# zzzzxxxx111/Rover-SLAM

Hardware: AMD Instinct MI355X
Metric: frames/s SuperPoint+LightGlue 640x480 (higher is better)
Workload: dtype f32; 1 GPU; configs[3] per GPU: 33 synthetic 640x480 u8 frames resident in HBM, SuperPoint extract (Kmax=1024, thr=0.0005) + LightGlue match of 32 consecutive pairs (9 layers, filter 0.1); 32 frames counted per GPU per step; seeded synthetic weights (centred descriptor head + calibrated LightGlue law, frames shifted by multiples of 8 px); the same resident frames every step (compute-bound path, no data-depend; frames_per_gpu=32, kmax=1024, lg_fold_wo=1, pairing=calibrated

## Files before the change

rover-slam_amd/csrc/gemm.hip:

```cpp
#include <stdlib.h>
#include "rfe_internal.h"

namespace rfe {

constexpr int BK = 32, LDT = BK + 1;

__device__ __forceinline__ float gelu_short(float t) {
    const float x = t * 0.70710678118654752f, ax = fabsf(x);
    const float k = __builtin_amdgcn_rcpf(fmaf(0.3275911f, ax, 1.0f));
    const float poly = fmaf(fmaf(fmaf(fmaf(1.061405429f, k, -1.453152027f), k, 1.421413741f), k, -0.284496736f), k, 0.254829592f) * k;
    const float er = 1.0f - poly * __builtin_amdgcn_exp2f(-(ax * ax) * 1.44269504088896341f);
    return 0.5f * t * (1.0f + copysignf(er, x));
}

typedef __attribute__((address_space(3))) void* gemm_lds_ptr_t;
typedef const __attribute__((address_space(1))) void* gemm_gptr_t;
template <int MB, int NB, bool RES, bool LNA = false, bool KP = false, bool ROPE = false>
__global__ __launch_bounds__(256, 2) void gemm_nt_kernel(GemmArgs g) {
    constexpr int BM = MB * 64, BN = NB * 64;
    constexpr int LDR = KP ? BK : LDT;
    static_assert(!KP || (!LNA && MB == 2), "KP: 128-row tiles without the fused LayerNorm only");
    static_assert(!ROPE || (KP && !RES && NB == 4), "ROPE: plain k-permuted 128 x 256 tile only");
    __shared__ __attribute__((aligned(16))) float lds_static[(BM + BN) * LDR];
    extern __shared__ __attribute__((aligned(16))) float lds_dynamic[];
// ... 287 lines not shown
        if (i < T) {
            const int r = i & 15;
            const int m = m0 + (wm * MB + (i >> 4)) * 32 + (r & 3) + 8 * (r >> 2) + 4 * h;
            if (m < M) {
                const int P = (int)gridDim.x * 2;
                float* sp = g.stats_out + (((size_t)m + (size_t)z * g.M) * P + bxt * 2 + wn) * 2;
                sp[0] = sm[0]; sp[1] = s2[0];
            }
        }
    }
}

bool gemm_nt_rope_ok(const GemmArgs& g) {
    const int batch = g.batch > 0 ? g.batch : 1;
    return g.kperm && batch == 1 && !g.m_valid && !g.R && !g.stats_in && !g.stats_out && !g.Bh && !g.relu && g.alpha == 1.0f && g.N % 256 == 0 &&
           g.rope_c0 % 256 == 0 && g.rope_c1 % 256 == 0 && (long long)((g.M + 127) / 128) * (g.N / 256) >= 256 && !gemm_latency_regime(g);
}

int launch_gemm_nt(hipStream_t s, const GemmArgs& g_in) {
    GemmArgs g = g_in;
    const int batch = g.batch > 0 ? g.batch : 1;
    auto tiles = [&](int bm, int bn) { return (long long)((g.M + bm - 1) / bm) * ((g.N + bn - 1) / bn) * batch; };
    if (g.rope_csn && !gemm_nt_rope_ok(g)) return -1;
    if (g.Bh && g.Bl && batch == 1 && !g.m_valid && !g.relu && g.N % 256 == 0 && g.K % 32 == 0 && (!g.A2 || g.K1 % 32 == 0) && tiles(128, 256) >= 256)
        return launch_gemm_h2(s, g);
    if (!g.rope_csn && gemm_latency_regime(g)) {
        if (launch_gemm_lat(s, g, nullptr, 0)) return 0;
    }
    const bool res = g.R != nullptr, lna = g.stats_in != nullptr;
    const bool kp = g.kperm != 0 && !lna;
#define RFE_GEMM_GO(MB_, NB_, GRID)                                                                  \
    do {                                                                                             \
        if (g.rope_csn && MB_ == 2 && NB_ == 4) {                                                    \
            static bool lr_[64]; ensure_dynamic_lds((const void*)gemm_nt_kernel<2, 4, false, false, true, true>, 128 * 64 * 4, lr_); \
            hipLaunchKernelGGL((gemm_nt_kernel<2, 4, false, false, true, true>), GRID, dim3(256), 128 * 64 * 4, s, g); \
        } else                                                                                       \
        if (kp && MB_ == 2) {                                                                        \
            if (res) hipLaunchKernelGGL((gemm_nt_kernel<MB_, NB_, true, false, MB_ == 2>), GRID, dim3(256), 0, s, g); \
            else hipLaunchKernelGGL((gemm_nt_kernel<MB_, NB_, false, false, MB_ == 2>), GRID, dim3(256), 0, s, g);    \
        } else                                                                                       \
        if (lna) hipLaunchKernelGGL((gemm_nt_kernel<MB_, NB_, true, true>), GRID, dim3(256), 0, s, g);   \
        else if (res) hipLaunchKernelGGL((gemm_nt_kernel<MB_, NB_, true>), GRID, dim3(256), 0, s, g);    \
        else hipLaunchKernelGGL((gemm_nt_kernel<MB_, NB_, false>), GRID, dim3(256), 0, s, g);        \
    } while (0)
    const bool big = (g.N % 256 == 0 && tiles(128, 256) >= 256) || tiles(128, 128) >= 256 || g.M > 8192;
    if (!big || g.N % 256) g.stats_out = nullptr;
    int ntiles;
    if (g.N % 256 == 0 && tiles(128, 256) >= 256) { ntiles = g.N / 256; RFE_GEMM_GO(2, 4, dim3(g.N / 256, (g.M + 127) / 128, batch)); }
    else if (tiles(128, 128) >= 256 || g.M > 8192) { ntiles = (g.N + 127) / 128; RFE_GEMM_GO(2, 2, dim3((g.N + 127) / 128, (g.M + 127) / 128, batch)); }
    else if (tiles(64, 128) >= 256) { ntiles = (g.N + 127) / 128; RFE_GEMM_GO(1, 2, dim3((g.N + 127) / 128, (g.M + 63) / 64, batch)); }
    else { ntiles = (g.N + 63) / 64; RFE_GEMM_GO(1, 1, dim3((g.N + 63) / 64, (g.M + 63) / 64, batch)); }
    return g.stats_out ? 2 * ntiles : 0;
}

}
```

rover-slam_amd/csrc/lg_kernels.hip:

```cpp
#include <stdlib.h>
#include "rfe_internal.h"

namespace rfe {

__global__ void lg_posenc_kernel(const float* __restrict__ kn, const float* __restrict__ wr, int rows, float2* __restrict__ csn) {
    const int gid = blockIdx.x * blockDim.x + threadIdx.x;
    if (gid >= rows * 32) return;
    const int i = gid >> 5, f = gid & 31;
    const float th = fmaf(wr[2 * f + 1], kn[2 * i + 1], wr[2 * f] * kn[2 * i]);
    csn[gid] = make_float2(cosf(th), sinf(th));
}
void launch_lg_posenc(hipStream_t s, const float* kn, const float* wr, int rows, float* csn) {
    hipLaunchKernelGGL(lg_posenc_kernel, dim3((rows * 32 + 255) / 256), dim3(256), 0, s, kn, wr, rows, reinterpret_cast<float2*>(csn));
}

constexpr int AT_Q = 128, AT_K = 64, AT_LDK = 65;
constexpr float AT_DEFER = 16.0f;
constexpr int AT_SPLIT_MAX = 8;
constexpr size_t AT_SPLIT_MAX_ROWS = 8192;

__device__ __forceinline__ float at_softmax_init(bool first, float m_run) { return first ? 0.f : -m_run; }
__device__ __forceinline__ void at_softmax_step(f32x16& st, bool first, float& m_run, float& l_run, f32x16& o0, f32x16& o1) {
    float mx = fmaxf(fmaxf(st[0], st[1]), st[2]);
#pragma unroll
// ... 332 lines not shown
            acc.x += o.x * w; acc.y += o.y * w; acc.z += o.z * w; acc.w += o.w * w;
        }
        const float inv = l > 0.f ? 1.0f / l : 0.f;
        acc.x *= inv; acc.y *= inv; acc.z *= inv; acc.w *= inv;
    }
    *reinterpret_cast<float4*>(out + row * 256 + head * 64 + d4 * 4) = acc;
}

size_t lg_attention_part_bytes(int nseq, int Lq) {
    const size_t rows = (size_t)nseq * Lq;
    return rows <= AT_SPLIT_MAX_ROWS ? rows * AT_SPLIT_MAX * (256 + 8) * sizeof(float) : 0;
}

constexpr int AT_PRIO = 1;
void launch_lg_attention(hipStream_t s, const float* q, const float* k, const float* v, int ld, float* out, int nseq, int Lq,
                         int Lk, const int* qlen, const int* klen, const int* kv_map, float* part, const float* rope_csn, bool fp16x2) {
    if (fp16x2 && (size_t)nseq * Lq >= 32768 && (ld % 4) == 0) {
        launch_lg_attention_h2(s, q, k, v, ld, out, nseq, Lq, Lk, qlen, klen, kv_map, rope_csn);
        return;
    }
    if (!rope_csn && (size_t)nseq * Lq <= AT_SPLIT_MAX_ROWS && launch_lg_attention_lat(s, q, k, v, ld, out, nseq, Lq, Lk, qlen, klen, kv_map, fp16x2)) return;
    const int nqb = (Lq + AT_Q - 1) / AT_Q;
    const int units8 = (4 * nseq + 7) / 8 * 8;
    const bool rope = rope_csn != nullptr;
    if (part && (size_t)nseq * Lq <= AT_SPLIT_MAX_ROWS) {
        const int units = nqb * 4 * nseq;
        int ns = 1;
        while (ns < AT_SPLIT_MAX && units * ns * 2 <= 256 && Lk / (ns * 2) >= 2 * AT_K) ns *= 2;
        if (ns > 1) {
            if (rope)
                hipLaunchKernelGGL((lg_attention_kernel<true, true>), dim3(nqb * units8, ns), dim3(256), 0, s, q, k, v, ld, out, Lq, Lk,
                                   nqb, qlen, klen, kv_map, AT_PRIO, part, nseq, rope_csn);
            else
                hipLaunchKernelGGL((lg_attention_kernel<true, false>), dim3(nqb * units8, ns), dim3(256), 0, s, q, k, v, ld, out, Lq, Lk,
                                   nqb, qlen, klen, kv_map, AT_PRIO, part, nseq, rope_csn);
            hipLaunchKernelGGL(lg_attention_combine_kernel, dim3((unsigned)(((size_t)nseq * Lq * 64 + 255) / 256)), dim3(256), 0, s, part,
                               ns, nseq, Lq, qlen, out);
            return;
        }
    }
    if (!rope && (ld % 4) == 0)
// ... 413 lines not shown
```

rover-slam_amd/csrc/rfe_api.hip:

```cpp
#include <stdio.h>
#include <stdlib.h>
#include <string.h>
#include <algorithm>
#include <map>
#include <mutex>
#include <tuple>
#include "rfe_internal.h"

using namespace rfe;

static std::string g_init_error;
static std::mutex g_mu;

namespace rfe {

int fail(rfe_ctx* c, int code, const std::string& msg) {
    if (c) c->err = msg;
    else { std::lock_guard<std::mutex> l(g_mu); g_init_error = msg; }
    return code;
}

int ensure_ws(rfe_ctx* c, void** p, size_t* cur, size_t need) {
    if (need <= *cur) return RFE_OK;
    if (*p) { RFE_HIP(c, hipStreamSynchronize(c->stream)); RFE_HIP(c, hipFree(*p)); *p = nullptr; *cur = 0; }
// ... 128 lines not shown
    hipDeviceProp_t prop;
    if ((e = hipGetDeviceProperties(&prop, device)) != hipSuccess)
        return fail(nullptr, RFE_ERR_HIP, std::string("hipGetDeviceProperties: ") + hipGetErrorString(e));
    if (strncmp(prop.gcnArchName, "gfx950", 6) != 0)
        return fail(nullptr, RFE_ERR_NO_DEVICE, std::string("rfe_init: kernels are built for gfx950 only, device is ") + prop.gcnArchName);
    rfe_ctx* c = new rfe_ctx();
    c->device = device;
    if ((e = hipStreamCreateWithFlags(&c->own_stream, hipStreamNonBlocking)) != hipSuccess) {
        delete c;
        return fail(nullptr, RFE_ERR_HIP, std::string("hipStreamCreate: ") + hipGetErrorString(e));
    }
    c->stream = c->own_stream;
    if ((e = hipStreamCreateWithFlags(&c->side_stream, hipStreamNonBlocking)) != hipSuccess ||
        (e = hipEventCreateWithFlags(&c->ev_fork, hipEventDisableTiming)) != hipSuccess ||
        (e = hipEventCreateWithFlags(&c->ev_join, hipEventDisableTiming)) != hipSuccess ||
        (e = hipEventCreateWithFlags(&c->ev_pyr, hipEventDisableTiming)) != hipSuccess) {
        rfe_destroy(c);
        return fail(nullptr, RFE_ERR_HIP, std::string("hipStreamCreate/hipEventCreate: ") + hipGetErrorString(e));
    }
    *out = c;
    return RFE_OK;
}

extern "C" void rfe_destroy(rfe_ctx* c) {
    if (!c) return;
    (void)hipSetDevice(c->device);
    (void)hipStreamSynchronize(c->stream);
    prof_collect(c);
    for (auto e : c->ev_pool) (void)hipEventDestroy(e);
    host_graph_release(c->g_extract);
    host_graph_release(c->g_match);
    auto fr = [](void* p) { if (p) (void)hipFree(p); };
    c->sp_hold.reset(); c->lg_hold.reset();
    fr(c->ws_sp); fr(c->ws_lg); fr(c->ws_io); fr(c->ws_tmp); fr(c->ws_st); fr(c->sp_cnt); fr(c->ws_pyr); fr(c->ws_ptab);
    if (c->h_pin) (void)hipHostFree(c->h_pin);
    if (c->side_stream) { (void)hipStreamSynchronize(c->side_stream); (void)hipStreamDestroy(c->side_stream); }
    if (c->ev_fork) (void)hipEventDestroy(c->ev_fork);
    if (c->ev_join) (void)hipEventDestroy(c->ev_join);
    if (c->ev_pyr) (void)hipEventDestroy(c->ev_pyr);
    (void)hipStreamDestroy(c->own_stream);
    delete c;
}

extern "C" int rfe_set_option(rfe_ctx* c, int option, int value) {
    if (!c) return RFE_ERR_INVALID;
    switch (option) {
        case RFE_OPT_LG_FOLD_WO: c->opt_lg_fold = value != 0; ++c->settings_gen; return RFE_OK;
        case RFE_OPT_LG_FP16X2: c->opt_lg_fp16x2 = value != 0; ++c->settings_gen; return RFE_OK;
        case RFE_OPT_HOST_GRAPH: c->opt_host_graph = value != 0; return RFE_OK;
        default: return fail(c, RFE_ERR_INVALID, "rfe_set_option: unknown option");
    }
}
extern "C" int rfe_get_option(rfe_ctx* c, int option, int* value) {
    if (!c || !value) return RFE_ERR_INVALID;
// ... 823 lines not shown
    b.x = a.take<float>(rows * 256); b.ctx = a.take<float>(rows * 256); b.msg = a.take<float>(rows * 256);
    b.md = a.take<float>(rows * 256);
    b.kn = a.take<float>(rows * 2); b.csn = a.take<float>(rows * 64); b.lnstat = a.take<float>(rows * 32);
    b.qkv = a.take<float>(rows * 768); b.h = a.take<float>(rows * 512); b.z = a.take<float>(rows);
    b.sim = a.take<float>((size_t)P * L * L);
    b.rowlse = a.take<float>((size_t)P * L); b.collse = a.take<float>((size_t)P * L); b.mx0 = a.take<float>((size_t)P * L);
    b.a0 = a.take<int32_t>((size_t)P * L); b.a1 = a.take<int32_t>((size_t)P * L);
    b.lens = a.take<int32_t>((size_t)2 * P); b.kvmap = a.take<int32_t>((size_t)2 * P);
    { const size_t pb = lg_attention_part_bytes(2 * P, L); b.apart = pb ? a.take<float>(pb / 4) : nullptr; }
    b.extra = a.take<char>(extra_bytes);
}

float* lg_part(const LgBuffers& b, int nseq, int L) { return (b.apart && lg_attention_part_bytes(nseq, L) > 0) ? b.apart : nullptr; }


void lg_ffn(rfe_ctx* c, LgBuffers& b, float* x, const float* second, int rows, const float* w1, const float* b1, const float* g,
            const float* be, const float* w2, const float* b2) {
    hipStream_t s = c->stream;
    int P = 0;
    { ProfScope p(c, "lg_ffn1");
      GemmArgs a = gemm_lgw(c, x, 256, w1, 512, b1, b.h, 512, rows, 512, 512);
      a.A2 = second; a.lda2 = 256; a.K1 = 256;
      if (!gemm_latency_regime(a)) a.stats_out = b.lnstat;
      P = launch_gemm_nt(s, a); }
    if (P == 0 && !c->opt_lg_fp16x2) {
        ProfScope p(c, "lg_ffn2");
        if (launch_ffn2_ln_lat(s, b.h, w2, b2, g, be, x, 256, x, 256, rows)) return;
    }
    if (P == 0) { ProfScope p(c, "lg_ln_gelu"); launch_lg_ln_gelu(s, b.h, g, be, rows); }
    { ProfScope p(c, "lg_ffn2");
      GemmArgs a = gemm_lgw(c, b.h, 512, w2, 512, b2, x, 256, rows, 256, 512);
      a.R = x; a.ldr = 256;
      if (P > 0) { a.stats_in = b.lnstat; a.stats_p = P; a.ln_g = g; a.ln_b = be; }
      launch_gemm_nt(s, a); }
}

bool lg_self_qkv_attention(rfe_ctx* c, LgBuffers& b, const LgLayerDev& Lw, const float* x, const float* csn, const int32_t* lens, int nseq, int L) {
    hipStream_t s = c->stream;
    const int rows = nseq * L;
    bool roped = false;
    { ProfScope p(c, "lg_qkv");
      GemmArgs a = gemm_lgw(c, x, 256, Lw.wqkv, 256, Lw.bqkv, b.qkv, 768, rows, 768, 256);
      if (gemm_latency_regime(a) && launch_gemm_lat(s, a, csn, 512)) roped = true;
      else {
          if (csn) {
              a.rope_c0 = 0; a.rope_c1 = 512;
              if (gemm_nt_rope_ok(a)) { a.rope_csn = csn; roped = true; }
          }
          launch_gemm_nt(s, a);
      } }
    { ProfScope p(c, "lg_attention");
      launch_lg_attention(s, b.qkv, b.qkv + 256, b.qkv + 512, 768, b.ctx, nseq, L, L, lens, lens, nullptr, lg_part(b, nseq, L), roped ? nullptr : csn, c->opt_lg_fp16x2); }
    return roped;
}

void lg_self_block(rfe_ctx* c, LgBuffers& b, const LgLayerDev& Lw, float* x, const float* csn, const int32_t* lens, int nseq, int L) {
    hipStream_t s = c->stream;
    const int rows = nseq * L;
    lg_self_qkv_attention(c, b, Lw, x, csn, lens, nseq, L);
    if (c->opt_lg_fold) {
        lg_ffn(c, b, x, b.ctx, rows, Lw.w1f, Lw.b1f, Lw.lng, Lw.lnb, Lw.w2, Lw.b2);
    } else {
        { ProfScope p(c, "lg_proj"); launch_gemm_nt(s, gemm_lgw(c, b.ctx, 256, Lw.wo, 256, Lw.bo, b.msg, 256, rows, 256, 256)); }
        lg_ffn(c, b, x, b.msg, rows, Lw.w1, Lw.b1, Lw.lng, Lw.lnb, Lw.w2, Lw.b2);
    }
}

int lg_forward(rfe_ctx* c, LgBuffers& b, int P, int L, float thr, int cap, int32_t* S, int32_t* pairs, float* ms,
               float* scores_opt, bool first_self_done = false, bool posenc_done = false) {
    hipStream_t s = c->stream;
    const LgWeightsDev& W = c->lg;
    const int rows = 2 * P * L, nseq = 2 * P;
    if (!first_self_done && !posenc_done) { ProfScope p(c, "lg_misc"); launch_lg_posenc(s, b.kn, W.wr, rows, b.csn); }
    for (int l = 0; l < LG_LAYERS; ++l) {
        const LgLayerDev& Lw = W.L[l];
        if (l > 0 || !first_self_done) lg_self_block(c, b, Lw, b.x, b.csn, b.lens, nseq, L);
        { ProfScope p(c, "lg_cross_qkv"); launch_gemm_nt(s, gemm_lgw(c, b.x, 256, Lw.cwqkv, 256, Lw.cbqkv, b.qkv, 512, rows, 512, 256)); }
        { ProfScope p(c, "lg_attention"); launch_lg_attention(s, b.qkv, b.qkv, b.qkv + 256, 512, b.ctx, nseq, L, L, b.lens, b.lens, b.kvmap, lg_part(b, nseq, L), nullptr, c->opt_lg_fp16x2); }
        if (c->opt_lg_fold) {
            lg_ffn(c, b, b.x, b.ctx, rows, Lw.cw1f, Lw.cb1f, Lw.clng, Lw.clnb, Lw.cw2, Lw.cb2);
        } else {
            { ProfScope p(c, "lg_proj"); launch_gemm_nt(s, gemm_lgw(c, b.ctx, 256, Lw.cwo, 256, Lw.cbo, b.msg, 256, rows, 256, 256)); }
            lg_ffn(c, b, b.x, b.msg, rows, Lw.cw1, Lw.cb1, Lw.clng, Lw.clnb, Lw.cw2, Lw.cb2);
        }
    }
    { ProfScope p(c, "lg_proj");
      GemmArgs a = gemm_lgw(c, b.x, 256, W.wp, 256, W.bp, b.md, 256, rows, 256, 256);
      a.alpha = 0.25f;
      launch_gemm_nt(s, a); }
    { ProfScope p(c, "lg_sim");
      GemmArgs g = gemm_lg(b.md, 256, b.md + (size_t)P * L * 256, 256, nullptr, b.sim, L, L, L, 256);
      g.batch = P; g.sA = (long long)L * 256; g.sB = (long long)L * 256; g.sC = (long long)L * L;
      g.m_valid = b.lens;
// ... 68 lines not shown

}

extern "C" int rfe_match_dev(rfe_ctx* c, const float* k0n, const float* k1n, const float* d0, const float* d1,
                             const int32_t* m, const int32_t* n, int P, int Mmax, int Nmax, float thr, int32_t* S,
                             int32_t* pairs, float* ms) {
    int rc = lg_check(c, P, Mmax, Nmax);
    if (rc) return rc;
    if (!k0n || !k1n || !d0 || !d1 || !m || !n || !S || !pairs || !ms) return fail(c, RFE_ERR_INVALID, "match: null pointer");
    RFE_HIP(c, hipSetDevice(c->device));
    const int L = ((std::max(Mmax, Nmax) + 3) / 4) * 4;
    if ((rc = ensure_ws(c, &c->ws_lg, &c->ws_lg_bytes, lg_ws_bytes(P, L)))) return rc;
    LgBuffers b;
    lg_carve(c->ws_lg, P, L, b);
    if ((rc = lg_stage(c, b, k0n, k1n, d0, d1, m, n, P, Mmax, Nmax, L))) return rc;
    return lg_forward(c, b, P, L, thr, std::min(Mmax, Nmax), S, pairs, ms, nullptr, false, true);
}

extern "C" int rfe_match(rfe_ctx* c, const float* k0n, const float* k1n, const float* d0, const float* d1,
                         const int32_t* m, const int32_t* n, int P, int Mmax, int Nmax, float thr, int32_t* S,
                         int32_t* pairs, float* ms) {
    int rc = lg_check(c, P, Mmax, Nmax);
    if (rc) return rc;
    if (!k0n || !k1n || !d0 || !d1 || !m || !n || !S || !pairs || !ms) return fail(c, RFE_ERR_INVALID, "match: null pointer");
    RFE_HIP(c, hipSetDevice(c->device));
    const int cap = std::min(Mmax, Nmax);
    const size_t bk0 = al((size_t)P * Mmax * 8), bk1 = al((size_t)P * Nmax * 8), bd0 = al((size_t)P * Mmax * 1024),
                 bd1 = al((size_t)P * Nmax * 1024), bi = al((size_t)P * 4), bp = al((size_t)P * cap * 8), bs = al((size_t)P * cap * 4);
    if ((rc = ensure_ws(c, &c->ws_io, &c->ws_io_bytes, bk0 + bk1 + bd0 + bd1 + 3 * bi + bp + bs))) return rc;
    char* p = (char*)c->ws_io;
    float* dk0 = (float*)p; p += bk0; float* dk1 = (float*)p; p += bk1; float* dd0 = (float*)p; p += bd0; float* dd1 = (float*)p; p += bd1;
// ... 59 lines not shown
    if ((rc = lg_check(c, B - 1, Kmax, Kmax))) return rc;
    if (!S || !pairs || !ms) return fail(c, RFE_ERR_INVALID, "stream: null match output");
    const int P = B - 1, L = ((Kmax + 3) / 4) * 4;
    const size_t kn_bytes = al((size_t)B * Kmax * 8);
    const size_t rot_bytes = al((size_t)B * L * 64 * 4);
    const size_t extra_bytes = kn_bytes + rot_bytes;
    if ((rc = ensure_ws(c, &c->ws_lg, &c->ws_lg_bytes, lg_ws_bytes(P, L, extra_bytes)))) return rc;
    LgBuffers b;
    lg_carve(c->ws_lg, P, L, b, extra_bytes);
    float* kn_all = (float*)b.extra;
    hipStream_t s = c->stream;
    if (L != Kmax) {
        { ProfScope p(c, "lg_misc");
          launch_normalize_kpts(s, kxy, (int64_t)B * Kmax, H, W, kn_all);
          if ((rc = lg_stage(c, b, kn_all, kn_all + (size_t)Kmax * 2, desc, desc + (size_t)Kmax * 256, n, n + 1, P, Kmax, Kmax, L))) return rc; }
        return lg_forward(c, b, P, L, filter_thr, Kmax, S, pairs, ms, nullptr, false, true);
    }
    float* xf = P == 1 ? b.x : b.md;
    float* csnf = P == 1 ? b.csn : (float*)(b.extra + kn_bytes);
    { ProfScope p(c, "lg_misc");
      launch_lg_frame_prologue(s, kxy, desc, c->lg.wr, n, B, L, H, W, kn_all, csnf, xf, b.lens, b.kvmap); }
    lg_self_block(c, b, c->lg.L[0], xf, csnf, n, B, L);
    if (P > 1) {
      ProfScope p(c, "lg_misc");
      const size_t half = (size_t)P * L;
      launch_copy_f32(s, xf, b.x, (int64_t)half * 256);
      launch_copy_f32(s, xf + (size_t)L * 256, b.x + half * 256, (int64_t)half * 256);
      launch_copy_f32(s, csnf, b.csn, (int64_t)half * 64);
      launch_copy_f32(s, csnf + (size_t)L * 64, b.csn + half * 64, (int64_t)half * 64); }
    RFE_HIP(c, hipGetLastError());
    return lg_forward(c, b, P, L, filter_thr, Kmax, S, pairs, ms, nullptr, true);
}

extern "C" int rfe_stereo_match_dev(rfe_ctx* c, const uint8_t* imgL, const uint8_t* imgR, int H, int W, int stride,
                                    const float* kL, int N, const float* kR, int Nr, const float* dL, const float* dR,
                                    float mb, float mbf, float* uRight, float* depth) {
    if (!c) return RFE_ERR_INVALID;
    if (N < 0 || Nr < 0 || N > 4096 || H <= 0 || W <= 0 || stride < W || !(mb > 0.f)) return fail(c, RFE_ERR_INVALID, "stereo_match: bad argument (0 <= N <= 4096, mb > 0, stride >= W)");
    if (N == 0) return RFE_OK;
    if (!imgL || !imgR || !kL || !dL || !uRight || !depth || (Nr > 0 && (!kR || !dR))) return fail(c, RFE_ERR_INVALID, "stereo_match: null pointer");
    RFE_HIP(c, hipSetDevice(c->device));
    int rc = ensure_ws(c, &c->ws_tmp, &c->ws_tmp_bytes, al((size_t)N * 4));
    if (rc) return rc;
    ProfScope p(c, "stereo_match");
    launch_stereo_match(c->stream, imgL, imgR, H, W, stride, kL, N, kR, Nr, dL, dR, mb, mbf, uRight, depth, (int32_t*)c->ws_tmp);
    RFE_HIP(c, hipGetLastError());
// ... 113 lines not shown
      launch_stereo_match_counts(ss, imgL, imgR, H, W, stride, kxy, kxy + (size_t)Kmax * 2, Kmax, n, desc,
                                 desc + (size_t)Kmax * 256, mb, mbf, uRight, depth, sadv); }
    if (st_fork) RFE_HIP(c, hipEventRecord(c->ev_join, ss));
    struct JoinGuard { rfe_ctx* c; hipStream_t s; bool on; ~JoinGuard() { if (on) (void)hipStreamWaitEvent(s, c->ev_join, 0); } } join_guard{c, s, st_fork};
    {
        const int L = ((Kmax + 3) / 4) * 4;
        if ((rc = ensure_ws(c, &c->ws_lg, &c->ws_lg_bytes, lg_ws_bytes(1, L)))) return rc;
        LgBuffers b;
        lg_carve(c->ws_lg, 1, L, b);
        const float sx = (float)W / 2, sy = (float)H / 2, scale = (float)(H > W ? H : W) / 2;
        { ProfScope ps(c, "lg_misc");
          hipLaunchKernelGGL(st_stage_kernel, dim3((unsigned)((2 * L + 3) / 4)), dim3(256), 0, s, kxy, desc, n, Kmax, L, sx, sy, scale, kn_slot[prev], desc_slot[prev],
                             n_slot[prev], c->st_have_prev ? 1 : 0, c->lg.wr, b.x, b.kn, reinterpret_cast<float2*>(b.csn), b.lens, b.kvmap, kn_slot[next], desc_slot[next],
                             n_slot[next]); }
        if (c->st_have_prev) {
            if ((rc = lg_forward(c, b, 1, L, filter_thr, Kmax, S, pairs, ms, nullptr, false, true))) return rc;
        } else {
            hipLaunchKernelGGL(st_zero_count_kernel, dim3(1), dim3(1), 0, s, S);
        }
    }
    c->st_flip = next;
    if (st_fork) { join_guard.on = false; RFE_HIP(c, hipStreamWaitEvent(s, c->ev_join, 0)); }
    c->st_have_prev = true;
    RFE_HIP(c, hipGetLastError());
    return RFE_OK;
}

namespace {

int stereo_pyr_table(rfe_ctx* c, int H, int W, int L, float sf, int sad_source, float mb, StereoPyrTable& T, size_t& frame) {
    int32_t h[RFE_MAX_LEVELS], w[RFE_MAX_LEVELS]; float sc[RFE_MAX_LEVELS];
// ... 113 lines not shown
    if (st_fork) { RFE_HIP(c, hipEventRecord(c->ev_fork, s)); RFE_HIP(c, hipStreamWaitEvent(ss, c->ev_fork, 0)); }
    { ProfScope ps(c, "stereo_match", ss);
      launch_stereo_match_pyr(ss, lv, lv + frame, T, kpts, octave, K, kpts + (size_t)K * 2, octave + K, K, n, desc, desc + (size_t)K * 256, mb, mbf,
                              sad_source == RFE_STEREO_SAD_LEVEL0, uRight, depth, sadv); }
    if (st_fork) RFE_HIP(c, hipEventRecord(c->ev_join, ss));
    struct JoinGuard { rfe_ctx* c; hipStream_t s; bool on; ~JoinGuard() { if (on) (void)hipStreamWaitEvent(s, c->ev_join, 0); } } join_guard{c, s, st_fork};
    {
        LgBuffers b;
        lg_carve(c->ws_lg, 1, L, b);
        const float sx = (float)W / 2, sy = (float)H / 2, scale = (float)(H > W ? H : W) / 2;
        { ProfScope ps(c, "lg_misc");
          hipLaunchKernelGGL(st_stage_f32_kernel, dim3((unsigned)((2 * L + 3) / 4)), dim3(256), 0, s, kpts, desc, n, K, L, sx, sy, scale, kn_slot[prev], desc_slot[prev],
                             n_slot[prev], c->st_have_prev ? 1 : 0, c->lg.wr, b.x, b.kn, reinterpret_cast<float2*>(b.csn), b.lens, b.kvmap, kn_slot[next], desc_slot[next],
                             n_slot[next]); }
        if (c->st_have_prev) {
            if ((rc = lg_forward(c, b, 1, L, filter_thr, K, S, pairs, ms, nullptr, false, true))) return rc;
        } else {
            hipLaunchKernelGGL(st_zero_count_kernel, dim3(1), dim3(1), 0, s, S);
        }
    }
    c->st_flip = next;
    if (st_fork) { join_guard.on = false; RFE_HIP(c, hipStreamWaitEvent(s, c->ev_join, 0)); }
    c->st_have_prev = true;
    RFE_HIP(c, hipGetLastError());
    return RFE_OK;
}

extern "C" int rfe_l2_distance_matrix_dev(rfe_ctx* c, const float* a, int M, const float* b, int N, float* out) {
    if (!c) return RFE_ERR_INVALID;
    if (M < 0 || N < 0 || (M > 0 && N > 0 && (!a || !b || !out))) return fail(c, RFE_ERR_INVALID, "l2_distance_matrix: bad argument");
    if (M == 0 || N == 0) return RFE_OK;
// ... 332 lines not shown
    if (rc) return rc;
    RFE_HIP(c, hipSetDevice(c->device));
    const int L = ((std::max(M, N) + 3) / 4) * 4, cap = std::min(M, N);
    const size_t extra = al((size_t)L * L * 4) + al(64) * 3 + al((size_t)cap * 8) + al((size_t)cap * 4);
    if ((rc = ensure_ws(c, &c->ws_lg, &c->ws_lg_bytes, lg_ws_bytes(1, L, extra)))) return rc;
    LgBuffers b;
    lg_carve(c->ws_lg, 1, L, b, extra);
    char* p = b.extra;
    float* sc = (float*)p; p += al((size_t)L * L * 4);
    int32_t* dm = (int32_t*)p; p += al(64); int32_t* dn = (int32_t*)p; p += al(64); int32_t* dS = (int32_t*)p; p += al(64);
    int32_t* dp = (int32_t*)p; p += al((size_t)cap * 8); float* dms = (float*)p;
    RFE_HIP(c, hipMemcpyAsync(dm, &M, 4, hipMemcpyHostToDevice, c->stream));
    RFE_HIP(c, hipMemcpyAsync(dn, &N, 4, hipMemcpyHostToDevice, c->stream));
    RFE_HIP(c, hipStreamSynchronize(c->stream));
    if ((rc = lg_stage(c, b, k0n, k1n, d0, d1, dm, dn, 1, M, N, L))) return rc;
    if ((rc = lg_forward(c, b, 1, L, 0.1f, cap, dS, dp, dms, scores ? sc : nullptr, false, true))) return rc;
    if (x0) RFE_HIP(c, hipMemcpyAsync(x0, b.x, (size_t)M * 1024, hipMemcpyDeviceToDevice, c->stream));
    if (x1) RFE_HIP(c, hipMemcpyAsync(x1, b.x + (size_t)L * 256, (size_t)N * 1024, hipMemcpyDeviceToDevice, c->stream));
    if (scores) RFE_HIP(c, hipMemcpy2DAsync(scores, (size_t)N * 4, sc, (size_t)L * 4, (size_t)N * 4, M, hipMemcpyDeviceToDevice, c->stream));
    RFE_HIP(c, hipStreamSynchronize(c->stream));
    return RFE_OK;
}
```

rover-slam_amd/csrc/rfe_internal.h:

```cpp
#pragma once
#include <hip/hip_runtime.h>
#include <stdint.h>
#include <stdlib.h>
#include <memory>
#include <string>
#include <vector>
#include "../../include/rover_fe.h"

typedef float f32x16 __attribute__((ext_vector_type(16)));
typedef float f32x4 __attribute__((ext_vector_type(4)));

namespace rfe {


struct SpLayer { int cin, cout, k; bool pool; };
static const SpLayer kSpLayers[12] = {
    {1, 64, 3, false}, {64, 64, 3, true}, {64, 64, 3, false}, {64, 64, 3, true}, {64, 128, 3, false}, {128, 128, 3, true},
    {128, 128, 3, false}, {128, 128, 3, false}, {128, 256, 3, false}, {256, 65, 1, false}, {128, 256, 3, false}, {256, 256, 1, false}};
enum { L_1A, L_1B, L_2A, L_2B, L_3A, L_3B, L_4A, L_4B, L_PA, L_PB, L_DA, L_DB };

constexpr int LG_LAYERS = 9;
constexpr int64_t SP_COUNT = 1300865;
constexpr int64_t LG_COUNT = 11321153;

// ... 29 lines not shown
    const float* A2; int lda2; int K1;
    const float* B; int ldb;
    const float* bias;
    const float* R; int ldr;
    float* C; int ldc;
    int M, N, K;
    float alpha; int relu;
    long long sA, sA2, sB, sC, sR;
    const int* m_valid;
    int batch;
    float* stats_out;
    const float* stats_in; int stats_p; const float* ln_g; const float* ln_b;
    const uint16_t* Bh; const uint16_t* Bl;
    int kperm;
    const float* rope_csn; int rope_c0, rope_c1;
};

}

inline rfe_hparams rfe_default_hparams() { return rfe_hparams{1024, 0.0005f, 4, 4, 0, rfe::LG_LAYERS, 4, 0.1f}; }

struct rfe_ctx {
    int device = 0;
    hipStream_t own_stream = nullptr;
    hipStream_t stream = nullptr;
    hipStream_t side_stream = nullptr;
    hipEvent_t ev_fork = nullptr, ev_join = nullptr;
    hipEvent_t ev_pyr = nullptr;
    std::string err;
    bool has_sp = false, has_lg = false;
    bool opt_lg_fold = true;
    bool opt_lg_fp16x2 = false;
    bool opt_host_graph = false;
    struct HostGraph {
        struct Slot { std::string key; hipGraphExec_t exec = nullptr; unsigned long long used = 0; };
        struct Seen { std::string key; int count = 0; unsigned long long used = 0; };
        Slot slot[4]; Seen seen[8]; unsigned long long tick = 0;
    };
    HostGraph g_extract, g_match;
    unsigned long long settings_gen = 0;
    rfe_hparams hp = rfe_default_hparams();
    rfe::SpWeightsDev sp;
    rfe::LgWeightsDev lg;
// ... 47 lines not shown
                          const float* b1a, const float* wp, const float* bias, float* out, long long frame_step = 0 );
inline void ensure_dynamic_lds(const void* kernel, int bytes, bool* done) {
    int dev = 0;
    (void)hipGetDevice(&dev);
    if (dev < 0 || dev >= 64 || !done[dev]) {
        (void)hipFuncSetAttribute(kernel, hipFuncAttributeMaxDynamicSharedMemorySize, bytes);
        if (dev >= 0 && dev < 64) done[dev] = true;
    }
}
int launch_gemm_h2(hipStream_t s, const GemmArgs& g);
void launch_split_f16(hipStream_t s, const float* x, uint16_t* hi, uint16_t* lo, size_t n);
bool gemm_nt_rope_ok(const GemmArgs& g);
int launch_gemm_nt(hipStream_t s, const GemmArgs& g);
inline bool gemm_latency_regime(const GemmArgs& g) {
    const long long b = g.batch > 0 ? g.batch : 1;
    auto tiles = [&](int bm, int bn) { return (long long)((g.M + bm - 1) / bm) * ((g.N + bn - 1) / bn) * b; };
    const bool big = (g.N % 256 == 0 && tiles(128, 256) >= 256) || tiles(128, 128) >= 256 || g.M > 8192;
    return !big;
}
bool launch_gemm_lat(hipStream_t s, const GemmArgs& g, const float* rope_csn, int rope_cols);
bool onnx_convert(const std::string& path, int kind, std::vector<float>& blob, rfe_hparams* hp, std::string& err);
bool launch_ffn2_ln_lat(hipStream_t s, const float* h, const float* w2, const float* b2, const float* ln_g, const float* ln_b, const float* R, int ldr,
                        float* C, int ldc, int M);
bool launch_lg_attention_lat(hipStream_t s, const float* q, const float* k, const float* v, int ld, float* out, int nseq, int Lq, int Lk,
                             const int* qlen, const int* klen, const int* kv_map, bool h2 = false );
void launch_softmax65_d2s(hipStream_t s, const float* logits, int ld, int B, int Hc, int Wc, float* score);
constexpr int NMS_MAX_RADIUS = 8;
void launch_nms(hipStream_t s, const float* score, int B, int H, int W, int radius , int border, float* tmp_ss,
                uint8_t* tmp_mask, uint8_t* tmp_supp, float* out);
void launch_select(hipStream_t s, const float* nms, int B, int H, int W, int Kmax, float thr,
                   float* cand_score, int32_t* cand_idx, int32_t* n_out, int32_t* kxy, float* score,
                   int32_t* chunk_cnt , bool topk_always ,
                   unsigned long long* sel_keys , int32_t* sel_n );
bool launch_sp_tail_lat(hipStream_t s, const float* logits, int B, int Hc, int Wc, int radius, int border, float thr, unsigned long long* cand_keys ,
                        int32_t* cand_cnt , float* smap_out , float* nmap_out );
void launch_select_keys(hipStream_t s, const unsigned long long* cand_keys, int32_t* cand_cnt, int B, int H, int W, int Kmax, bool topk_always,
                        int32_t* n_out, int32_t* kxy, float* score);
void launch_keys_from_map(hipStream_t s, const float* nms, int B, int HW, float thr, unsigned long long* cand_keys, int32_t* cand_cnt);
void launch_descmap_norm(hipStream_t s, float* dmap, int64_t cells);
void launch_desc_sample(hipStream_t s, const float* dmap, int B, int Hc, int Wc, int H, int W,
                        const int32_t* n, const int32_t* kxy, int Kmax, float* desc, uint8_t* desc_bin );
void launch_lg_posenc(hipStream_t s, const float* kn, const float* wr, int rows, float* csn );
void launch_lg_attention(hipStream_t s, const float* q, const float* k, const float* v, int ld ,
                         float* out, int nseq, int Lq, int Lk, const int* qlen, const int* klen,
                         const int* kv_map ,
                         float* part ,
                         const float* rope_csn = nullptr ,
                         bool fp16x2 = false );
void launch_lg_attention_h2(hipStream_t s, const float* q, const float* k, const float* v, int ld, float* out, int nseq, int Lq, int Lk,
                            const int* qlen, const int* klen, const int* kv_map, const float* rope_csn);
size_t lg_attention_part_bytes(int nseq, int Lq);
void launch_lg_ln_gelu(hipStream_t s, float* h, const float* g, const float* b, int64_t rows);
void launch_lg_assign(hipStream_t s, const float* sim, const float* z0, const float* z1, int P, int L,
                      int cap, const int* m, const int* n, float thr, float* scores_opt, float* rowlse,
                      float* collse, int32_t* a0, float* mx0, int32_t* a1, int32_t* S, int32_t* pairs,
                      float* ms, int scores_pair ,
                      const float* x, const float* wm, const float* bm, float* z );
bool lg_assign_few_pairs(int P, int L);
void launch_lg_frame_prologue(hipStream_t s, const int32_t* kxy, const float* desc, const float* wr, const int32_t* nkp, int B, int L, int rows, int cols,
                              float* kn, float* csn, float* x, int32_t* lens, int32_t* kvmap);
void launch_lg_matchability(hipStream_t s, const float* x, const float* w, const float* b, int64_t rows, float* z);
void launch_copy_f32(hipStream_t s, const float* src, float* dst, int64_t n);
void launch_normalize_kpts(hipStream_t s, const int32_t* kxy, int64_t n, int rows, int cols, float* out);
// ... 45 lines not shown
```

Before: 937.1 frames/s.

## Peel last frame of LightGlue layer 0 onto side stream and fold cross-QKV

Layer 0 of the multi-pair LightGlue path is split. The main stream runs the self block for the first P frames, while the final frame's self block and cross-QKV GEMM run concurrently on the side stream. The x/csn pair-duplication copies also move to the side stream. Cross-attention for layer 0 is now computed directly on per-frame QKV (two attention launches), so QKV is no longer recomputed on the duplicated pair layout. A route_M/route_nseq hint keeps the GEMM and attention kernel selection based on the full problem size, at the cost of extra events, stream synchronisation and buffer-aliasing complexity.

```diff
diff --git a/rover-slam_amd/csrc/gemm.hip b/rover-slam_amd/csrc/gemm.hip
--- a/rover-slam_amd/csrc/gemm.hip
+++ b/rover-slam_amd/csrc/gemm.hip
@@ -325,13 +325,14 @@
 bool gemm_nt_rope_ok(const GemmArgs& g) {
     const int batch = g.batch > 0 ? g.batch : 1;
     return g.kperm && batch == 1 && !g.m_valid && !g.R && !g.stats_in && !g.stats_out && !g.Bh && !g.relu && g.alpha == 1.0f && g.N % 256 == 0 &&
-           g.rope_c0 % 256 == 0 && g.rope_c1 % 256 == 0 && (long long)((g.M + 127) / 128) * (g.N / 256) >= 256 && !gemm_latency_regime(g);
+           g.rope_c0 % 256 == 0 && g.rope_c1 % 256 == 0 && (long long)((gemm_route_rows(g) + 127) / 128) * (g.N / 256) >= 256 && !gemm_latency_regime(g);
 }
 
 int launch_gemm_nt(hipStream_t s, const GemmArgs& g_in) {
     GemmArgs g = g_in;
     const int batch = g.batch > 0 ? g.batch : 1;
-    auto tiles = [&](int bm, int bn) { return (long long)((g.M + bm - 1) / bm) * ((g.N + bn - 1) / bn) * batch; };
+    const int RM = gemm_route_rows(g);
+    auto tiles = [&](int bm, int bn) { return (long long)((RM + bm - 1) / bm) * ((g.N + bn - 1) / bn) * batch; };
     if (g.rope_csn && !gemm_nt_rope_ok(g)) return -1;
     if (g.Bh && g.Bl && batch == 1 && !g.m_valid && !g.relu && g.N % 256 == 0 && g.K % 32 == 0 && (!g.A2 || g.K1 % 32 == 0) && tiles(128, 256) >= 256)
         return launch_gemm_h2(s, g);
@@ -354,11 +355,11 @@
         else if (res) hipLaunchKernelGGL((gemm_nt_kernel<MB_, NB_, true>), GRID, dim3(256), 0, s, g);    \
         else hipLaunchKernelGGL((gemm_nt_kernel<MB_, NB_, false>), GRID, dim3(256), 0, s, g);        \
     } while (0)
-    const bool big = (g.N % 256 == 0 && tiles(128, 256) >= 256) || tiles(128, 128) >= 256 || g.M > 8192;
+    const bool big = (g.N % 256 == 0 && tiles(128, 256) >= 256) || tiles(128, 128) >= 256 || RM > 8192;
     if (!big || g.N % 256) g.stats_out = nullptr;
     int ntiles;
     if (g.N % 256 == 0 && tiles(128, 256) >= 256) { ntiles = g.N / 256; RFE_GEMM_GO(2, 4, dim3(g.N / 256, (g.M + 127) / 128, batch)); }
-    else if (tiles(128, 128) >= 256 || g.M > 8192) { ntiles = (g.N + 127) / 128; RFE_GEMM_GO(2, 2, dim3((g.N + 127) / 128, (g.M + 127) / 128, batch)); }
+    else if (tiles(128, 128) >= 256 || RM > 8192) { ntiles = (g.N + 127) / 128; RFE_GEMM_GO(2, 2, dim3((g.N + 127) / 128, (g.M + 127) / 128, batch)); }
     else if (tiles(64, 128) >= 256) { ntiles = (g.N + 127) / 128; RFE_GEMM_GO(1, 2, dim3((g.N + 127) / 128, (g.M + 63) / 64, batch)); }
     else { ntiles = (g.N + 63) / 64; RFE_GEMM_GO(1, 1, dim3((g.N + 63) / 64, (g.M + 63) / 64, batch)); }
     return g.stats_out ? 2 * ntiles : 0;
diff --git a/rover-slam_amd/csrc/lg_kernels.hip b/rover-slam_amd/csrc/lg_kernels.hip
--- a/rover-slam_amd/csrc/lg_kernels.hip
+++ b/rover-slam_amd/csrc/lg_kernels.hip
@@ -370,17 +370,19 @@
 
 constexpr int AT_PRIO = 1;
 void launch_lg_attention(hipStream_t s, const float* q, const float* k, const float* v, int ld, float* out, int nseq, int Lq,
-                         int Lk, const int* qlen, const int* klen, const int* kv_map, float* part, const float* rope_csn, bool fp16x2) {
-    if (fp16x2 && (size_t)nseq * Lq >= 32768 && (ld % 4) == 0) {
+                         int Lk, const int* qlen, const int* klen, const int* kv_map, float* part, const float* rope_csn, bool fp16x2, int route_nseq) {
+    const int rseq = route_nseq > 0 ? route_nseq : nseq;
+    const size_t rrows = (size_t)rseq * Lq;
+    if (fp16x2 && rrows >= 32768 && (ld % 4) == 0) {
         launch_lg_attention_h2(s, q, k, v, ld, out, nseq, Lq, Lk, qlen, klen, kv_map, rope_csn);
         return;
     }
-    if (!rope_csn && (size_t)nseq * Lq <= AT_SPLIT_MAX_ROWS && launch_lg_attention_lat(s, q, k, v, ld, out, nseq, Lq, Lk, qlen, klen, kv_map, fp16x2)) return;
+    if (!rope_csn && rrows <= AT_SPLIT_MAX_ROWS && launch_lg_attention_lat(s, q, k, v, ld, out, nseq, Lq, Lk, qlen, klen, kv_map, fp16x2)) return;
     const int nqb = (Lq + AT_Q - 1) / AT_Q;
     const int units8 = (4 * nseq + 7) / 8 * 8;
     const bool rope = rope_csn != nullptr;
-    if (part && (size_t)nseq * Lq <= AT_SPLIT_MAX_ROWS) {
-        const int units = nqb * 4 * nseq;
+    if (part && rrows <= AT_SPLIT_MAX_ROWS) {
+        const int units = nqb * 4 * rseq;
         int ns = 1;
         while (ns < AT_SPLIT_MAX && units * ns * 2 <= 256 && Lk / (ns * 2) >= 2 * AT_K) ns *= 2;
         if (ns > 1) {
diff --git a/rover-slam_amd/csrc/rfe_api.hip b/rover-slam_amd/csrc/rfe_api.hip
--- a/rover-slam_amd/csrc/rfe_api.hip
+++ b/rover-slam_amd/csrc/rfe_api.hip
@@ -166,7 +166,9 @@
     if ((e = hipStreamCreateWithFlags(&c->side_stream, hipStreamNonBlocking)) != hipSuccess ||
         (e = hipEventCreateWithFlags(&c->ev_fork, hipEventDisableTiming)) != hipSuccess ||
         (e = hipEventCreateWithFlags(&c->ev_join, hipEventDisableTiming)) != hipSuccess ||
-        (e = hipEventCreateWithFlags(&c->ev_pyr, hipEventDisableTiming)) != hipSuccess) {
+        (e = hipEventCreateWithFlags(&c->ev_pyr, hipEventDisableTiming)) != hipSuccess ||
+        (e = hipEventCreateWithFlags(&c->ev_lg_self, hipEventDisableTiming)) != hipSuccess ||
+        (e = hipEventCreateWithFlags(&c->ev_lg_x, hipEventDisableTiming)) != hipSuccess) {
         rfe_destroy(c);
         return fail(nullptr, RFE_ERR_HIP, std::string("hipStreamCreate/hipEventCreate: ") + hipGetErrorString(e));
     }
@@ -190,6 +192,8 @@
     if (c->ev_fork) (void)hipEventDestroy(c->ev_fork);
     if (c->ev_join) (void)hipEventDestroy(c->ev_join);
     if (c->ev_pyr) (void)hipEventDestroy(c->ev_pyr);
+    if (c->ev_lg_self) (void)hipEventDestroy(c->ev_lg_self);
+    if (c->ev_lg_x) (void)hipEventDestroy(c->ev_lg_x);
     (void)hipStreamDestroy(c->own_stream);
     delete c;
 }
@@ -1043,33 +1047,36 @@
 float* lg_part(const LgBuffers& b, int nseq, int L) { return (b.apart && lg_attention_part_bytes(nseq, L) > 0) ? b.apart : nullptr; }
 
 
+struct LgSlice { hipStream_t on = nullptr; int whole_seq = 0; };
+
 void lg_ffn(rfe_ctx* c, LgBuffers& b, float* x, const float* second, int rows, const float* w1, const float* b1, const float* g,
-            const float* be, const float* w2, const float* b2) {
-    hipStream_t s = c->stream;
+            const float* be, const float* w2, const float* b2, hipStream_t on = nullptr, int route_rows = 0 ) {
+    hipStream_t s = on ? on : c->stream;
     int P = 0;
-    { ProfScope p(c, "lg_ffn1");
+    { ProfScope p(c, "lg_ffn1", s);
       GemmArgs a = gemm_lgw(c, x, 256, w1, 512, b1, b.h, 512, rows, 512, 512);
-      a.A2 = second; a.lda2 = 256; a.K1 = 256;
+      a.A2 = second; a.lda2 = 256; a.K1 = 256; a.route_M = route_rows;
       if (!gemm_latency_regime(a)) a.stats_out = b.lnstat;
       P = launch_gemm_nt(s, a); }
     if (P == 0 && !c->opt_lg_fp16x2) {
-        ProfScope p(c, "lg_ffn2");
+        ProfScope p(c, "lg_ffn2", s);
         if (launch_ffn2_ln_lat(s, b.h, w2, b2, g, be, x, 256, x, 256, rows)) return;
     }
-    if (P == 0) { ProfScope p(c, "lg_ln_gelu"); launch_lg_ln_gelu(s, b.h, g, be, rows); }
-    { ProfScope p(c, "lg_ffn2");
+    if (P == 0) { ProfScope p(c, "lg_ln_gelu", s); launch_lg_ln_gelu(s, b.h, g, be, rows); }
+    { ProfScope p(c, "lg_ffn2", s);
       GemmArgs a = gemm_lgw(c, b.h, 512, w2, 512, b2, x, 256, rows, 256, 512);
-      a.R = x; a.ldr = 256;
+      a.R = x; a.ldr = 256; a.route_M = route_rows;
       if (P > 0) { a.stats_in = b.lnstat; a.stats_p = P; a.ln_g = g; a.ln_b = be; }
       launch_gemm_nt(s, a); }
 }
 
-bool lg_self_qkv_attention(rfe_ctx* c, LgBuffers& b, const LgLayerDev& Lw, const float* x, const float* csn, const int32_t* lens, int nseq, int L) {
-    hipStream_t s = c->stream;
+bool lg_self_qkv_attention(rfe_ctx* c, LgBuffers& b, const LgLayerDev& Lw, const float* x, const float* csn, const int32_t* lens, int nseq, int L, LgSlice sl = {}) {
+    hipStream_t s = sl.on ? sl.on : c->stream;
     const int rows = nseq * L;
     bool roped = false;
-    { ProfScope p(c, "lg_qkv");
+    { ProfScope p(c, "lg_qkv", s);
       GemmArgs a = gemm_lgw(c, x, 256, Lw.wqkv, 256, Lw.bqkv, b.qkv, 768, rows, 768, 256);
+      a.route_M = sl.whole_seq * L;
       if (gemm_latency_regime(a) && launch_gemm_lat(s, a, csn, 512)) roped = true;
       else {
           if (csn) {
@@ -1078,34 +1085,47 @@
           }
           launch_gemm_nt(s, a);
       } }
-    { ProfScope p(c, "lg_attention");
-      launch_lg_attention(s, b.qkv, b.qkv + 256, b.qkv + 512, 768, b.ctx, nseq, L, L, lens, lens, nullptr, lg_part(b, nseq, L), roped ? nullptr : csn, c->opt_lg_fp16x2); }
+    { ProfScope p(c, "lg_attention", s);
+      launch_lg_attention(s, b.qkv, b.qkv + 256, b.qkv + 512, 768, b.ctx, nseq, L, L, lens, lens, nullptr, lg_part(b, sl.whole_seq ? sl.whole_seq : nseq, L),
+                          roped ? nullptr : csn, c->opt_lg_fp16x2, sl.whole_seq); }
     return roped;
 }
 
-void lg_self_block(rfe_ctx* c, LgBuffers& b, const LgLayerDev& Lw, float* x, const float* csn, const int32_t* lens, int nseq, int L) {
-    hipStream_t s = c->stream;
-    const int rows = nseq * L;
-    lg_self_qkv_attention(c, b, Lw, x, csn, lens, nseq, L);
+void lg_self_block(rfe_ctx* c, LgBuffers& b, const LgLayerDev& Lw, float* x, const float* csn, const int32_t* lens, int nseq, int L, LgSlice sl = {}) {
+    hipStream_t s = sl.on ? sl.on : c->stream;
+    const int rows = nseq * L, route = sl.whole_seq * L;
+    lg_self_qkv_attention(c, b, Lw, x, csn, lens, nseq, L, sl);
     if (c->opt_lg_fold) {
-        lg_ffn(c, b, x, b.ctx, rows, Lw.w1f, Lw.b1f, Lw.lng, Lw.lnb, Lw.w2, Lw.b2);
+        lg_ffn(c, b, x, b.ctx, rows, Lw.w1f, Lw.b1f, Lw.lng, Lw.lnb, Lw.w2, Lw.b2, s, route);
     } else {
-        { ProfScope p(c, "lg_proj"); launch_gemm_nt(s, gemm_lgw(c, b.ctx, 256, Lw.wo, 256, Lw.bo, b.msg, 256, rows, 256, 256)); }
-        lg_ffn(c, b, x, b.msg, rows, Lw.w1, Lw.b1, Lw.lng, Lw.lnb, Lw.w2, Lw.b2);
-    }
-}
+        { ProfScope p(c, "lg_proj", s);
+          GemmArgs a = gemm_lgw(c, b.ctx, 256, Lw.wo, 256, Lw.bo, b.msg, 256, rows, 256, 256);
+          a.route_M = route;
+          launch_gemm_nt(s, a); }
+        lg_ffn(c, b, x, b.msg, rows, Lw.w1, Lw.b1, Lw.lng, Lw.lnb, Lw.w2, Lw.b2, s, route);
+    }
+}
+
+enum LgLayer0 {
+    LG_L0_NONE = 0,
+    LG_L0_SELF,
+    LG_L0_CROSS_ATTENTION
+};
 
 int lg_forward(rfe_ctx* c, LgBuffers& b, int P, int L, float thr, int cap, int32_t* S, int32_t* pairs, float* ms,
-               float* scores_opt, bool first_self_done = false, bool posenc_done = false) {
+               float* scores_opt, LgLayer0 l0_done = LG_L0_NONE, bool posenc_done = false, hipEvent_t x_ready = nullptr) {
     hipStream_t s = c->stream;
     const LgWeightsDev& W = c->lg;
     const int rows = 2 * P * L, nseq = 2 * P;
+    const bool first_self_done = l0_done != LG_L0_NONE;
     if (!first_self_done && !posenc_done) { ProfScope p(c, "lg_misc"); launch_lg_posenc(s, b.kn, W.wr, rows, b.csn); }
     for (int l = 0; l < LG_LAYERS; ++l) {
         const LgLayerDev& Lw = W.L[l];
         if (l > 0 || !first_self_done) lg_self_block(c, b, Lw, b.x, b.csn, b.lens, nseq, L);
-        { ProfScope p(c, "lg_cross_qkv"); launch_gemm_nt(s, gemm_lgw(c, b.x, 256, Lw.cwqkv, 256, Lw.cbqkv, b.qkv, 512, rows, 512, 256)); }
-        { ProfScope p(c, "lg_attention"); launch_lg_attention(s, b.qkv, b.qkv, b.qkv + 256, 512, b.ctx, nseq, L, L, b.lens, b.lens, b.kvmap, lg_part(b, nseq, L), nullptr, c->opt_lg_fp16x2); }
+        if (l > 0 || l0_done != LG_L0_CROSS_ATTENTION) {
+            { ProfScope p(c, "lg_cross_qkv"); launch_gemm_nt(s, gemm_lgw(c, b.x, 256, Lw.cwqkv, 256, Lw.cbqkv, b.qkv, 512, rows, 512, 256)); }
+            { ProfScope p(c, "lg_attention"); launch_lg_attention(s, b.qkv, b.qkv, b.qkv + 256, 512, b.ctx, nseq, L, L, b.lens, b.lens, b.kvmap, lg_part(b, nseq, L), nullptr, c->opt_lg_fp16x2); }
+        } else if (x_ready) RFE_HIP(c, hipStreamWaitEvent(s, x_ready, 0));
         if (c->opt_lg_fold) {
             lg_ffn(c, b, b.x, b.ctx, rows, Lw.cw1f, Lw.cb1f, Lw.clng, Lw.clnb, Lw.cw2, Lw.cb2);
         } else {
@@ -1204,7 +1224,7 @@
     LgBuffers b;
     lg_carve(c->ws_lg, P, L, b);
     if ((rc = lg_stage(c, b, k0n, k1n, d0, d1, m, n, P, Mmax, Nmax, L))) return rc;
-    return lg_forward(c, b, P, L, thr, std::min(Mmax, Nmax), S, pairs, ms, nullptr, false, true);
+    return lg_forward(c, b, P, L, thr, std::min(Mmax, Nmax), S, pairs, ms, nullptr, LG_L0_NONE, true);
 }
 
 extern "C" int rfe_match(rfe_ctx* c, const float* k0n, const float* k1n, const float* d0, const float* d1,
@@ -1294,22 +1314,55 @@
         { ProfScope p(c, "lg_misc");
           launch_normalize_kpts(s, kxy, (int64_t)B * Kmax, H, W, kn_all);
           if ((rc = lg_stage(c, b, kn_all, kn_all + (size_t)Kmax * 2, desc, desc + (size_t)Kmax * 256, n, n + 1, P, Kmax, Kmax, L))) return rc; }
-        return lg_forward(c, b, P, L, filter_thr, Kmax, S, pairs, ms, nullptr, false, true);
+        return lg_forward(c, b, P, L, filter_thr, Kmax, S, pairs, ms, nullptr, LG_L0_NONE, true);
     }
     float* xf = P == 1 ? b.x : b.md;
     float* csnf = P == 1 ? b.csn : (float*)(b.extra + kn_bytes);
     { ProfScope p(c, "lg_misc");
       launch_lg_frame_prologue(s, kxy, desc, c->lg.wr, n, B, L, H, W, kn_all, csnf, xf, b.lens, b.kvmap); }
-    lg_self_block(c, b, c->lg.L[0], xf, csnf, n, B, L);
-    if (P > 1) {
-      ProfScope p(c, "lg_misc");
-      const size_t half = (size_t)P * L;
-      launch_copy_f32(s, xf, b.x, (int64_t)half * 256);
-      launch_copy_f32(s, xf + (size_t)L * 256, b.x + half * 256, (int64_t)half * 256);
-      launch_copy_f32(s, csnf, b.csn, (int64_t)half * 64);
-      launch_copy_f32(s, csnf + (size_t)L * 64, b.csn + half * 64, (int64_t)half * 64); }
+    const LgLayerDev& L0 = c->lg.L[0];
+    if (P == 1) {
+        lg_self_block(c, b, L0, xf, csnf, n, B, L);
+        RFE_HIP(c, hipGetLastError());
+        return lg_forward(c, b, P, L, filter_thr, Kmax, S, pairs, ms, nullptr, LG_L0_SELF);
+    }
+    hipStream_t ss = c->side_stream;
+    const bool peel = P % 32 == 0 && (size_t)B * L > 8192 && !c->opt_lg_fp16x2;
+    const int nmain = peel ? P : B;
+    const size_t row0 = (size_t)P * L;
+    float* cq = b.qkv + (peel ? (size_t)B * L * 768 : 0);
+    auto cross_qkv = [&](hipStream_t on, size_t r0, int nrows) {
+        ProfScope p(c, "lg_cross_qkv", on);
+        GemmArgs a = gemm_lgw(c, xf + r0 * 256, 256, L0.cwqkv, 256, L0.cbqkv, cq + r0 * 512, 512, nrows, 512, 256);
+        a.route_M = 2 * P * L;
+        launch_gemm_nt(on, a);
+    };
+    if (peel) { RFE_HIP(c, hipEventRecord(c->ev_fork, s)); RFE_HIP(c, hipStreamWaitEvent(ss, c->ev_fork, 0)); }
+    lg_self_block(c, b, L0, xf, csnf, n, nmain, L, LgSlice{s, B});
+    cross_qkv(s, 0, nmain * L);
+    RFE_HIP(c, hipEventRecord(c->ev_lg_self, s));
+    if (peel) {
+        LgBuffers bl = b;
+        bl.qkv += row0 * 768; bl.ctx += row0 * 256; bl.msg += row0 * 256; bl.h += row0 * 512; bl.lnstat += row0 * 32;
+        lg_self_block(c, bl, L0, xf + row0 * 256, csnf + row0 * 64, n + P, 1, L, LgSlice{ss, B});
+        cross_qkv(ss, row0, L);
+        RFE_HIP(c, hipEventRecord(c->ev_join, ss));
+    }
+    RFE_HIP(c, hipStreamWaitEvent(ss, c->ev_lg_self, 0));
+    { ProfScope p(c, "lg_misc", ss);
+      launch_copy_f32(ss, xf, b.x, (int64_t)row0 * 256);
+      launch_copy_f32(ss, xf + (size_t)L * 256, b.x + row0 * 256, (int64_t)row0 * 256);
+      launch_copy_f32(ss, csnf, b.csn, (int64_t)row0 * 64);
+      launch_copy_f32(ss, csnf + (size_t)L * 64, b.csn + row0 * 64, (int64_t)row0 * 64); }
+    RFE_HIP(c, hipEventRecord(c->ev_lg_x, ss));
+    if (peel) RFE_HIP(c, hipStreamWaitEvent(s, c->ev_join, 0));
+    { ProfScope p(c, "lg_attention");
+      float* part = lg_part(b, 2 * P, L);
+      const float* f1 = cq + (size_t)L * 512;
+      launch_lg_attention(s, cq, f1, f1 + 256, 512, b.ctx, P, L, L, b.lens, b.lens + P, nullptr, part, nullptr, c->opt_lg_fp16x2, 2 * P);
+      launch_lg_attention(s, f1, cq, cq + 256, 512, b.ctx + row0 * 256, P, L, L, b.lens + P, b.lens, nullptr, part, nullptr, c->opt_lg_fp16x2, 2 * P); }
     RFE_HIP(c, hipGetLastError());
-    return lg_forward(c, b, P, L, filter_thr, Kmax, S, pairs, ms, nullptr, true);
+    return lg_forward(c, b, P, L, filter_thr, Kmax, S, pairs, ms, nullptr, LG_L0_CROSS_ATTENTION, false, c->ev_lg_x);
 }
 
 extern "C" int rfe_stereo_match_dev(rfe_ctx* c, const uint8_t* imgL, const uint8_t* imgR, int H, int W, int stride,
@@ -1453,7 +1506,7 @@
                              n_slot[prev], c->st_have_prev ? 1 : 0, c->lg.wr, b.x, b.kn, reinterpret_cast<float2*>(b.csn), b.lens, b.kvmap, kn_slot[next], desc_slot[next],
                              n_slot[next]); }
         if (c->st_have_prev) {
-            if ((rc = lg_forward(c, b, 1, L, filter_thr, Kmax, S, pairs, ms, nullptr, false, true))) return rc;
+            if ((rc = lg_forward(c, b, 1, L, filter_thr, Kmax, S, pairs, ms, nullptr, LG_L0_NONE, true))) return rc;
         } else {
             hipLaunchKernelGGL(st_zero_count_kernel, dim3(1), dim3(1), 0, s, S);
         }
@@ -1597,7 +1650,7 @@
                              n_slot[prev], c->st_have_prev ? 1 : 0, c->lg.wr, b.x, b.kn, reinterpret_cast<float2*>(b.csn), b.lens, b.kvmap, kn_slot[next], desc_slot[next],
                              n_slot[next]); }
         if (c->st_have_prev) {
-            if ((rc = lg_forward(c, b, 1, L, filter_thr, K, S, pairs, ms, nullptr, false, true))) return rc;
+            if ((rc = lg_forward(c, b, 1, L, filter_thr, K, S, pairs, ms, nullptr, LG_L0_NONE, true))) return rc;
         } else {
             hipLaunchKernelGGL(st_zero_count_kernel, dim3(1), dim3(1), 0, s, S);
         }
@@ -1960,7 +2013,7 @@
     RFE_HIP(c, hipMemcpyAsync(dn, &N, 4, hipMemcpyHostToDevice, c->stream));
     RFE_HIP(c, hipStreamSynchronize(c->stream));
     if ((rc = lg_stage(c, b, k0n, k1n, d0, d1, dm, dn, 1, M, N, L))) return rc;
-    if ((rc = lg_forward(c, b, 1, L, 0.1f, cap, dS, dp, dms, scores ? sc : nullptr, false, true))) return rc;
+    if ((rc = lg_forward(c, b, 1, L, 0.1f, cap, dS, dp, dms, scores ? sc : nullptr, LG_L0_NONE, true))) return rc;
     if (x0) RFE_HIP(c, hipMemcpyAsync(x0, b.x, (size_t)M * 1024, hipMemcpyDeviceToDevice, c->stream));
     if (x1) RFE_HIP(c, hipMemcpyAsync(x1, b.x + (size_t)L * 256, (size_t)N * 1024, hipMemcpyDeviceToDevice, c->stream));
     if (scores) RFE_HIP(c, hipMemcpy2DAsync(scores, (size_t)N * 4, sc, (size_t)L * 4, (size_t)N * 4, M, hipMemcpyDeviceToDevice, c->stream));
diff --git a/rover-slam_amd/csrc/rfe_internal.h b/rover-slam_amd/csrc/rfe_internal.h
--- a/rover-slam_amd/csrc/rfe_internal.h
+++ b/rover-slam_amd/csrc/rfe_internal.h
@@ -67,7 +67,9 @@
     const uint16_t* Bh; const uint16_t* Bl;
     int kperm;
     const float* rope_csn; int rope_c0, rope_c1;
-};
+    int route_M;
+};
+inline int gemm_route_rows(const GemmArgs& g) { return g.route_M > 0 ? g.route_M : g.M; }
 
 }
 
@@ -80,6 +82,7 @@
     hipStream_t side_stream = nullptr;
     hipEvent_t ev_fork = nullptr, ev_join = nullptr;
     hipEvent_t ev_pyr = nullptr;
+    hipEvent_t ev_lg_self = nullptr, ev_lg_x = nullptr;
     std::string err;
     bool has_sp = false, has_lg = false;
     bool opt_lg_fold = true;
@@ -157,8 +160,9 @@
 int launch_gemm_nt(hipStream_t s, const GemmArgs& g);
 inline bool gemm_latency_regime(const GemmArgs& g) {
     const long long b = g.batch > 0 ? g.batch : 1;
-    auto tiles = [&](int bm, int bn) { return (long long)((g.M + bm - 1) / bm) * ((g.N + bn - 1) / bn) * b; };
-    const bool big = (g.N % 256 == 0 && tiles(128, 256) >= 256) || tiles(128, 128) >= 256 || g.M > 8192;
+    const int M = gemm_route_rows(g);
+    auto tiles = [&](int bm, int bn) { return (long long)((M + bm - 1) / bm) * ((g.N + bn - 1) / bn) * b; };
+    const bool big = (g.N % 256 == 0 && tiles(128, 256) >= 256) || tiles(128, 128) >= 256 || M > 8192;
     return !big;
 }
 bool launch_gemm_lat(hipStream_t s, const GemmArgs& g, const float* rope_csn, int rope_cols);
@@ -189,7 +193,8 @@
                          const int* kv_map ,
                          float* part ,
                          const float* rope_csn = nullptr ,
-                         bool fp16x2 = false );
+                         bool fp16x2 = false ,
+                         int route_nseq = 0 );
 void launch_lg_attention_h2(hipStream_t s, const float* q, const float* k, const float* v, int ld, float* out, int nseq, int Lq, int Lk,
                             const int* qlen, const int* klen, const int* kv_map, const float* rope_csn);
 size_t lg_attention_part_bytes(int nseq, int Lq);
```

New measurement: 942.0 frames/s, median of 6. Within noise of the previous version (+0.5%).
